# ericlingit/jieba-go

Measured on AMD Instinct MI355X. Metric: UTF-8 Chinese chars/sec segmented (whole node) + achieved HBM GB/s vs peak, higher is better.
Workload: dtype f64

## Files before the change

jieba-go_amd/csrc/jb_kernels.hip:

```cpp
#include <type_traits>

#include "jb_kdev.h"
#include "jb_kstages.h"

#include <algorithm>

namespace jb {

#define START_B (-0.26268660809250016)
#define START_S (-1.4652633398537678)
#define T_BE (-0.51082562376599)
#define T_BM (-0.916290731874155)
#define T_EB (-0.5897149736854513)
#define T_ES (-0.8085250474669937)
#define T_ME (-0.33344856811948514)
#define T_MM (-1.2603623820268226)
#define T_SB (-0.7211965654669841)
#define T_SS (-0.6658631448798212)

__global__ void k_docbits(const uint64_t* __restrict__ doc_off, uint32_t ndocs, uint64_t nbytes,
                          uint32_t* __restrict__ bits, uint32_t* __restrict__ counters,
                          uint64_t* __restrict__ tstat, uint32_t ntt) {
    const uint32_t d = blockIdx.x * blockDim.x + threadIdx.x;
    if (d < CNT_ALL) counters[d] = 0u;
    if (d < ntt) tstat[d] = 0ull;
    if (d >= ndocs) return;
    const uint64_t o = doc_off[d];
    if (o < nbytes) atomicOr(bits + (o >> 5), 1u << (o & 31u));
}

constexpr uint32_t kTileE = kTileBytes / 3 + 2;
constexpr uint32_t kLA = 8;
constexpr uint32_t kLABytes = 40;
constexpr uint32_t kTileEX = kTileE + kLA;
constexpr uint32_t kMwStage = kTileBytes + 64u;
constexpr uint32_t kMwOffE = kTileEX * 8u;
constexpr uint32_t kMwOffDb = kMwOffE + kTileEX * 4u;
constexpr uint32_t kMwOffWl = kMwOffDb + (kTileBytes / 32u + 3u) * 4u;
constexpr uint32_t kMwOffScan = (kMwOffWl + kTileE * 2u + 3u) & ~3u;
constexpr uint32_t kMwSortB = 64u;
constexpr uint32_t kMwOffHist = kMwOffScan + 8u * 4u;
constexpr uint32_t kMwLds = kMwOffHist + kMwSortB * 4u;
constexpr uint32_t kMwOffHot = (kMwOffE + 15u) & ~15u;
static_assert(kMwOffHot % 16u == 0u && kMwOffHot + 10u * JB_HOT_SLOTS <= kMwOffDb && JB_HOT_SLOTS == 512u,
              "k_mark_walk: the hot rows fit under the entry list, 256 threads stage them");
static_assert(kMwOffE >= kMwStage, "staged text must fit under the entry cells");
static_assert(kTileBytes + kLABytes + 4u <= kMwStage - 16u && kTileBytes + kLABytes + 4u <= kTileBytes + 64u,
              "lookahead bytes are staged and have document bits");
static_assert(kMwLds + 16u <= 163840u / 8u, "k_mark_walk: 8 workgroups per CU");

constexpr uint32_t kEntCont = 0x40000000u;
constexpr uint32_t kEntEdge = 0x80000000u;
__device__ __forceinline__ uint32_t ent_code(uint32_t e) { return e & 0x1FFFFu; }
__device__ __forceinline__ uint32_t ent_pos(uint32_t e) { return (e >> 18) & 0xFFFu; }
__device__ __forceinline__ uint32_t ent_w(uint32_t e) { return 3u + ((e >> 17) & 1u); }

#ifndef JB_MW_SGPR
#define JB_MW_SGPR 80
#endif
#ifndef JB_MW_WALKS
#define JB_MW_WALKS 1
#endif
#define JB_MW_ATTR __attribute__((amdgpu_num_sgpr(JB_MW_SGPR), amdgpu_waves_per_eu(8, 8)))
__global__ __launch_bounds__(256) JB_MW_ATTR void k_mark_walk(const uint8_t* __restrict__ text, uint64_t nbytes,
                                                   const uint32_t* __restrict__ docbits, DevImage im,
                                                   uint32_t* __restrict__ lanemask, uint2* __restrict__ tile_cnt,
                                                   uint64_t* __restrict__ erec, uint32_t* __restrict__ tile4,
                                                   uint64_t* __restrict__ alnum16, uint32_t* __restrict__ sbits,
                                                   uint32_t* __restrict__ ebits, uint32_t diag,
                                                   uint64_t* __restrict__ dbg, uint32_t split) {
    __shared__ __attribute__((aligned(16))) uint8_t s_raw[kMwLds];
    uint64_t* const s_c = reinterpret_cast<uint64_t*>(s_raw);
    uint8_t* const s_t = s_raw;
    uint32_t* const s_e = reinterpret_cast<uint32_t*>(s_raw + kMwOffE);
    uint32_t* const s_db = reinterpret_cast<uint32_t*>(s_raw + kMwOffDb);
    uint16_t* const s_wl = reinterpret_cast<uint16_t*>(s_raw + kMwOffWl);
    uint32_t* const lds = reinterpret_cast<uint32_t*>(s_raw + kMwOffScan);
    __shared__ uint32_t s_nla, s_nwl;
#if JB_STAMPS
    const bool stamps = (diag & 0x100u) != 0;
#else
    const bool stamps = false;
#endif
    uint64_t c0 = stamps ? __builtin_amdgcn_s_memtime() : 0, c1 = 0, c2 = 0, c3 = 0, c0b = 0, c1b = 0;
    uint32_t trips = 0;
    const uint32_t tile = blockIdx.x >> split, part = blockIdx.x & ((1u << split) - 1u);
    const uint64_t t0 = (uint64_t)tile * kTileBytes;
    static_assert(kMwStage / 16 > 256u && kMwStage / 16 <= 512u, "the staged text is two loads per thread at most");
    uint4 va = make_uint4(0, 0, 0, 0), vb = make_uint4(0, 0, 0, 0);
    {
        const int64_t g = (int64_t)t0 - 16 + 16 * (int64_t)threadIdx.x, g2 = g + 16 * 256;
        if (g >= 0 && (uint64_t)g + 16 <= nbytes + 64) va = *reinterpret_cast<const uint4*>(text + g);
        if (threadIdx.x < kMwStage / 16 - 256u && (uint64_t)g2 + 16 <= nbytes + 64)
            vb = *reinterpret_cast<const uint4*>(text + g2);
    }
    const uint4 hv4 = reinterpret_cast<const uint4*>(im.hot)[threadIdx.x];
    const uint32_t ht2 = reinterpret_cast<const uint32_t*>(im.hot + JB_HOT_SLOTS)[threadIdx.x];
    const uint64_t lastw = (nbytes + 31) >> 5;
    uint32_t dbw = 0;
    if (threadIdx.x < kTileBytes / 32 + 3) {
        const uint64_t wi = (t0 >> 5) + threadIdx.x;
        dbw = wi < lastw ? docbits[wi] : 0u;
    }
    if (threadIdx.x == 0) {
        s_nla = 0;
        s_nwl = 0;
    }
    uint32_t* const s_hist = reinterpret_cast<uint32_t*>(s_raw + kMwOffHist);
    if (threadIdx.x < kMwSortB) s_hist[threadIdx.x] = 0u;
    const uint64_t p0 = t0 + threadIdx.x * 16u;
    uint64_t M;
    {
        const int64_t base = (int64_t)p0 - 4;
        if (base >= 0) {
            const uint64_t wi = (uint64_t)base >> 5;
            const uint32_t off = (uint32_t)base & 31u;
            const uint64_t lo = wi < lastw ? docbits[wi] : 0u;
            const uint64_t hi = wi + 1 < lastw ? docbits[wi + 1] : 0u;
            M = ((hi << 32) | lo) >> off;
        } else {
            M = (uint64_t)docbits[0] << 4;
        }
        if (nbytes < p0 + 20) {
            const int64_t endk = (int64_t)nbytes - base;
            if (endk <= 0) M = ~0ull;
            else M |= ~0ull << endk;
        }
    }
    reinterpret_cast<uint4*>(s_t)[threadIdx.x] = va;
    if (threadIdx.x < kMwStage / 16 - 256u) reinterpret_cast<uint4*>(s_t)[threadIdx.x + 256u] = vb;
    if (threadIdx.x < kTileBytes / 32 + 3) s_db[threadIdx.x] = dbw;
    reinterpret_cast<uint4*>(s_raw + kMwOffHot)[threadIdx.x] = hv4;
    reinterpret_cast<uint32_t*>(s_raw + kMwOffHot + 8u * JB_HOT_SLOTS)[threadIdx.x] = ht2;
    {
        const uint64_t wz = (t0 >> 5) + (threadIdx.x & 127u);
        if (wz < lastw + 2u) __builtin_nontemporal_store(0u, (threadIdx.x < 128u ? sbits : ebits) + wz);
    }
    __syncthreads();
    if (stamps) c0b = __builtin_amdgcn_s_memtime();
    const uint8_t* win = s_t + 12 + threadIdx.x * 16u;
    uint32_t xw[5];
    {
        const uint4 v4 = *reinterpret_cast<const uint4*>(win + 4);
        xw[1] = v4.x;
        xw[2] = v4.y;
        xw[3] = v4.z;
        xw[4] = v4.w;
        uint32_t w0 = 0;
        if ((threadIdx.x & 63u) == 0u) w0 = reinterpret_cast<const uint32_t*>(win)[0];
        xw[0] = (uint32_t)__builtin_amdgcn_update_dpp((int)w0, (int)xw[4], 0x138, 0xF, 0xF, false);
    }
    {
        const bool al = ((uint32_t)jb_any_alnum4(xw[1]) | (uint32_t)jb_any_alnum4(xw[2]) |
                         (uint32_t)jb_any_alnum4(xw[3]) | (uint32_t)jb_any_alnum4(xw[4])) != 0u;
        const uint64_t am = __ballot(al);
        if ((threadIdx.x & 63u) == 0) alnum16[(t0 >> 10) + (threadIdx.x >> 6)] = am;
    }
    uint32_t lead = 0;
#pragma unroll
    for (int j = 0; j < 5; j++) {
        const uint32_t x = xw[j];
        const uint32_t f = (x & (x << 1) & 0x80808080u) >> 7;
        lead |= ((f * 0x204081u) >> 21 & 0xFu) << (4 * j);
    }
    uint32_t covered = 0, hanb = 0;
    uint64_t cl[7];
    uint32_t hsm = 0, kp = 0;
    uint32_t rowp[4] = {0u, 0u, 0u, 0u};
    {
        constexpr uint64_t k3000 = (1ull << 5) | (1ull << 7) | (0x1FFull << 0x21) | (0xFull << 0x38);
        uint32_t l = lead, slow = 0, xs[7], vm = 0;
        uint64_t kq = 0;
#pragma unroll
        for (int i = 0; i < 7; i++) {
            vm |= (l != 0u ? 1u : 0u) << i;
            const uint32_t k = l ? (uint32_t)__builtin_ctz(l) : 0u;
            kq |= (uint64_t)k << (5 * i);
            xs[i] = lds4(win, k);
            l &= l - 1u;
        }
#pragma unroll
        for (int i = 0; i < 7; i++) {
            const bool v = (vm >> i) & 1u;
            const uint32_t k = (uint32_t)(kq >> (5 * i)) & 31u, x = xs[i];
            const uint32_t b0 = x & 0xFFu;
            const uint32_t r = ((b0 & 0x0Fu) << 12) | (((x >> 8) & 0x3Fu) << 6) | ((x >> 16) & 0x3Fu);
            const bool plain = (b0 - 0xE1u < 12u) | (b0 - 0xEEu < 2u);
            const bool rare = (r - 0x2E80u < 0x180u) | (r - 0xF900u < 0x200u);
            const bool ok = ((x & 0x00C0C000u) == 0x00808000u) & (((uint32_t)(M >> (k + 1u)) & 3u) == 0u);
            const uint32_t o = r - 0x3000u;
            const bool h = (r - 0x4E00u <= 0x9FFCu - 0x4E00u) | (r - 0x3400u <= 0x4DBFu - 0x3400u) |
                           ((o < 64u) & (((k3000 >> (o & 63u)) & 1ull) != 0ull));
            const bool fast = plain & !(ok & rare);
            slow |= ((v & !fast) ? 1u : 0u) << k;
            covered |= ((v & fast & ok) ? 3u : 0u) << (k + 1u);
            hanb |= ((v & fast & ok & h) ? 7u : 0u) << k;
            const bool dr = v & fast & ok & h & (k >= 4u) & (r >= JB_DIRECT_LO);
            rowp[i >> 1] |= (dr ? r - 0x3300u : 0u) << (16 * (i & 1));
            hsm |= (dr ? 1u : 0u) << i;
            kp |= (dr ? k - 4u : 0u) << (4 * i);
        }
        slow |= l;
        lead = slow;
    }
    while (lead) {
        const uint32_t k = __builtin_ctz(lead);
        lead &= lead - 1u;
        const uint32_t lim = 1u + (uint32_t)__builtin_ctzll(((M >> (k + 1)) & 7ull) | 8ull);
        uint32_t r;
        const uint32_t w = dec_lead(lds4(win, k), lim, &r);
        covered |= ((1u << (w - 1u)) - 1u) << (k + 1u);
        if (w >= 3u && han_cp(r)) hanb |= ((1u << w) - 1u) << k;
    }
    if (p0 == 0) hanb &= ~0xFu;
    uint32_t valid = 0xFFFF0u;
    if (nbytes < p0 + 16) valid = nbytes > p0 ? ((1u << (uint32_t)(nbytes - p0)) - 1u) << 4 : 0u;
    const uint32_t bs = ~covered & valid & ((uint32_t)M | (hanb ^ (hanb << 1)));
    const uint32_t bmask = (bs >> 4) & 0xFFFFu, zmask = ((bs & hanb) >> 4) & 0xFFFFu;
    __builtin_nontemporal_store(bmask | (zmask << 16), lanemask + tile * 256u + threadIdx.x);
    uint32_t tot;
    block_scan_u32(__popc(bmask) | (__popc(zmask) << 16), lds, &tot);
    if (threadIdx.x == 0) tile_cnt[tile] = make_uint2(tot & 0xFFFFu, tot >> 16);
    if (stamps) c1 = __builtin_amdgcn_s_memtime();

    uint32_t hs = ((hanb & ~covered & valid) >> 4) & 0xFFFFu;
    {
        const uint64_t* s_hv = reinterpret_cast<const uint64_t*>(s_raw + kMwOffHot);
        const uint16_t* s_ht = reinterpret_cast<const uint16_t*>(s_raw + kMwOffHot + 8u * JB_HOT_SLOTS);
        uint32_t hit = 0, tg[7];
#pragma unroll
        for (int i = 0; i < 7; i++) {
            const uint32_t r = ((rowp[i >> 1] >> (16 * (i & 1))) & 0xFFFFu) + 0x3300u;
            tg[i] = s_ht[jb_hot_slot(r)];
            cl[i] = s_hv[jb_hot_slot(r)];
        }
#pragma unroll
        for (int i = 0; i < 7; i++) {
            const uint32_t r = ((rowp[i >> 1] >> (16 * (i & 1))) & 0xFFFFu) + 0x3300u;
            hit |= (((hsm >> i) & 1u) & (tg[i] == r ? 1u : 0u)) << i;
        }
#pragma unroll
        for (int i = 0; i < 7; i++) {
            const uint32_t row = (rowp[i >> 1] >> (16 * (i & 1))) & 0xFFFFu;
            if (!((hit >> i) & 1u)) cl[i] = 0ull;
            if ((~hit & hsm) >> i & 1u) cl[i] = im.l1row[row];
        }
    }
    uint32_t nent;
    uint32_t o = block_scan_u32(__popc(hs), lds, &nent);
    bool has4 = false;
    {
        uint32_t w4m = 0;
        if (__popc(hs) != __popc(hsm)) {
            const uint32_t ne = __popc(hs);
            uint32_t h2 = hs;
            hsm = 0;
            kp = 0;
#pragma unroll
            for (int i = 0; i < 6; i++) {
                cl[i] = 0ull;
                if ((uint32_t)i < ne) {
                    const uint32_t k = (uint32_t)__builtin_ctz(h2);
                    h2 &= h2 - 1u;
                    const uint32_t x = lds4(win, k + 4u);
                    const uint32_t r = (x & 0xF0u) == 0xE0u
                                           ? ((x & 0x0Fu) << 12) | (((x >> 8) & 0x3Fu) << 6) | ((x >> 16) & 0x3Fu)
                                           : ((x & 0x07u) << 18) | (((x >> 8) & 0x3Fu) << 12) |
                                                 (((x >> 16) & 0x3Fu) << 6) | ((x >> 24) & 0x3Fu);
                    cl[i] = im.l1row[jb_row(im.pagemap, r)];
                    hsm |= 1u << i;
                    kp |= k << (4 * i);
                    w4m |= (r >= 0x10000u ? 1u : 0u) << i;
                }
            }
            cl[6] = 0ull;
        }
        has4 = w4m != 0u;
        const uint32_t top = hsm ? 31u - (uint32_t)__builtin_clz(hsm) : 0u;
        const uint32_t lastend =
            hsm ? ((kp >> (4u * top)) & 15u) + 4u + 3u + ((w4m >> top) & 1u) : 0u;
        const uint32_t le255 = __builtin_amdgcn_readlane(lastend, 63);
        const bool la = threadIdx.x >= 192u && le255 >= 20u;
        uint32_t law = 0, lar = 0, lacd = 0;
        if (la) {
            const uint32_t j = threadIdx.x & 63u, q = kTileBytes + j;
            if (j < kLABytes) {
                const uint64_t db = ((((uint64_t)s_db[(q >> 5) + 1u]) << 32) | s_db[q >> 5]) >> (q & 31u);
                uint32_t lim = 1u + (uint32_t)__builtin_ctzll(((db >> 1) & 7ull) | 8ull);
                const uint64_t gq = t0 + q;
                if (gq + lim > nbytes) lim = gq < nbytes ? (uint32_t)(nbytes - gq) : 0u;
                lar = (db & 1ull) ? 0u : han_rune(lds4(s_t, q + 16u), lim, &law);
            }
            lacd = lar ? rune_code(im, lar) : 0u;
        }
#pragma unroll
        for (int i = 0; i < 7; i++) {
            if ((hsm >> i) & 1u)
                s_e[o + __popc(hsm & ((1u << i) - 1u))] = jb_l1row_code(cl[i]) | (((w4m >> i) & 1u) << 17) |
                                                          ((threadIdx.x * 16u + ((kp >> (4 * i)) & 15u)) << 18);
            cl[i] = ((hsm >> i) & 1u) ? jb_l1row_cell(cl[i]) : 0ull;
        }
        if (la) {
            const uint32_t j = threadIdx.x & 63u;
            const uint32_t w = law, r = lar, cdj = lacd;
            const uint64_t hm = __ballot(r != 0u), w4b = __ballot(w == 4u);
            uint64_t chain = 0;
            uint32_t jj = le255 - 20u, n = 0;
            bool go = true;
#pragma unroll
            for (int i = 0; i < (int)kLA; i++) {
                if (go && jj < kLABytes && ((hm >> jj) & 1ull)) {
                    chain |= 1ull << jj;
                    n++;
                    jj += ((w4b >> jj) & 1ull) ? 4u : 3u;
                } else {
                    go = false;
                }
            }
            if ((chain >> j) & 1ull) {
                const uint32_t ix = (uint32_t)__popcll(chain & ((1ull << j) - 1ull));
                s_e[nent + ix] = cdj | ((w == 4u ? 1u : 0u) << 17) | (ix + 1u < n ? kEntCont : (go ? kEntEdge : 0u));
            }
            if (j == 0u) s_nla = n;
        }
        __syncthreads();
        if (stamps) c1b = __builtin_amdgcn_s_memtime();
#pragma unroll
        for (int i = 0; i < 7; i++)
            if ((hsm >> i) & 1u) s_c[o + __popc(hsm & ((1u << i) - 1u))] = cl[i];
    }
    __syncthreads();
    const uint32_t nla = s_nla;
    uint32_t wm = 0;
    for (uint32_t i = threadIdx.x, k = 0; i < nent; i += 256u, k++) {
        const uint32_t e = s_e[i];
        const uint32_t nxt = ent_pos(e) + ent_w(e);
        uint32_t f = 0;
        if (nxt >= kTileBytes) f = nla ? kEntCont : 0u;
        else if (i + 1u < nent && ent_pos(s_e[i + 1u]) == nxt && !((s_db[nxt >> 5] >> (nxt & 31u)) & 1u)) f = kEntCont;
        s_e[i] = e | f;
        const uint64_t c1 = s_c[i];
        const uint32_t fc = jb_cell_fc(c1), wi = jb_cell_widx(c1);
        uint64_t r1 = 0;
        bool go = false;
        if (jb_cell_check(c1) != JB_CHECK_ROOT) {
            r1 = 1ull | ((uint64_t)(JB_WIDX_ABSENT + 1u) << kRecTop);
        } else if (wi > kRecIdxMax && fc != JB_FC_NEG) {
            r1 = 0ull;
        } else if (fc == JB_FC_ZERO) {
            r1 = 1ull | ((uint64_t)(wi + 1u) << kRecTop);
        } else {
            if (fc == JB_FC_POS) r1 = 1ull | ((uint64_t)(wi + 1u) << kRecTop);
            go = jb_cell_hc(c1) != 0u && f != 0u;
        }
        if (!im.plainw) {
            r1 = 0ull;
            go = false;
        }
        if (!go) {
            s_c[i] = r1;
        } else if (i < ((nent * part) >> split) || i >= ((nent * (part + 1u)) >> split)) {
        } else {
            const uint32_t ln = (jb_cell_base(c1) + ent_code(s_e[i + 1u])) >> 4;
            const uint32_t b = (ln * 0x9E3779B1u) >> 26;
            static_assert(kMwSortB == 64u && kTileEX <= 2048u, "bucket (6 bits) and rank (11 bits) in the check field");
            const uint32_t rk = atomicAdd(&s_hist[b], 1u);
            s_c[i] = (c1 & ~0x3FFFFFull) | (b << 11) | rk;
            wm |= 1u << k;
        }
    }
    const int any4 = __syncthreads_or(has4);
    if (threadIdx.x == 0) tile4[tile] = any4 ? 1u : 0u;
    if (threadIdx.x < 64u) {
        const uint32_t h = s_hist[threadIdx.x];
        const uint32_t x = wave_incl_scan(h);
        s_hist[threadIdx.x] = x - h;
        if (threadIdx.x == 63u) s_nwl = x;
    }
    __syncthreads();
    for (uint32_t k = 0; wm >> k; k++) {
        if ((wm >> k) & 1u) {
            const uint32_t i = threadIdx.x + 256u * k;
            const uint32_t ck = (uint32_t)s_c[i] & 0x3FFFFFu;
            s_wl[s_hist[ck >> 11] + (ck & 2047u)] = (uint16_t)i;
        }
    }
    __syncthreads();
    if (stamps) c2 = __builtin_amdgcn_s_memtime();
    const uint32_t* ent = s_e;
    const uint32_t wv = threadIdx.x >> 6;
    const uint32_t nwl = s_nwl;
    uint32_t head = (nwl * wv) >> 2;
    const uint32_t hi = (nwl * (wv + 1u)) >> 2;
    struct Walk {
        bool act, ovf;
        uint32_t j, js, id, base, len, nedge, m, en;
        uint64_t rw;
    };
    Walk wk[JB_MW_WALKS];
#pragma unroll
    for (int q = 0; q < JB_MW_WALKS; q++) {
        wk[q].act = wk[q].ovf = false;
        wk[q].j = wk[q].js = wk[q].id = wk[q].base = wk[q].len = wk[q].nedge = wk[q].m = wk[q].en = 0u;
        wk[q].rw = 0ull;
    }
    for (;;) {
#pragma unroll
        for (int q = 0; q < JB_MW_WALKS; q++) {
            Walk& w = wk[q];
            const uint64_t need = __ballot(!w.act);
            const uint32_t rank =
                __builtin_amdgcn_mbcnt_hi((uint32_t)(need >> 32), __builtin_amdgcn_mbcnt_lo((uint32_t)need, 0u));
            const uint32_t j0 = head + rank;
            const bool fresh = !w.act && j0 < hi;
            head = min(hi, head + (uint32_t)__popcll(need));
            if (fresh) {
                w.js = s_wl[j0];
                w.j = w.js;
                const uint64_t c = s_c[w.j];
                w.id = ent_code(ent[w.j]);
                w.base = jb_cell_base(c);
                const bool pos = jb_cell_fc(c) == JB_FC_POS;
                w.m = pos ? 1u : 0u;
                w.nedge = w.m;
                w.rw = pos ? (uint64_t)(jb_cell_widx(c) + 1u) << kRecTop : 0ull;
                w.len = 1u;
                w.ovf = false;
                w.act = true;
                w.en = ent[w.j + 1u];
            }
        }
        uint64_t child[JB_MW_WALKS];
        uint32_t tt[JB_MW_WALKS], en2[JB_MW_WALKS];
#pragma unroll
        for (int q = 0; q < JB_MW_WALKS; q++) {
            tt[q] = wk[q].base + ent_code(wk[q].en);
            child[q] = wk[q].act ? im.cells[tt[q]] : 0ull;
            en2[q] = ent[wk[q].j + 2u];
        }
#pragma unroll
        for (int q = 0; q < JB_MW_WALKS; q++) {
            Walk& w = wk[q];
            if (w.act) {
                const uint64_t ch = child[q];
                const bool hit = dat_hit(ch, w.id);
                ++w.len;
                const uint32_t wi = jb_cell_widx(ch);
                const bool pos = hit && jb_cell_fc(ch) == JB_FC_POS;
                const bool bad = pos && (w.len > kEdgeMaxL || w.nedge >= 4u || wi > kRecIdxMax);
                const bool add = pos && !bad;
                w.ovf |= bad;
                w.m |= add ? 1u << ((w.len - 1u) & 7u) : 0u;
                w.rw = add ? (w.rw >> kEdgeIdxBits) | ((uint64_t)(wi + 1u) << kRecTop) : w.rw;
                w.nedge += add ? 1u : 0u;
                const bool more = hit && jb_cell_hc(ch) && !w.ovf;
                const bool go = more && (w.en & kEntCont);
                const bool dfr = more && !(w.en & kEntCont) && (w.en & kEntEdge);
                ++w.j;
                w.en = en2[q];
                w.id = tt[q];
                w.base = jb_cell_base(ch);
                if (!go) {
                    s_c[w.js] = (w.ovf || dfr) ? 0ull : ((uint64_t)w.m | w.rw);
                    w.act = false;
                }
            }
        }
        trips++;
        bool any = false;
#pragma unroll
        for (int q = 0; q < JB_MW_WALKS; q++) any |= wk[q].act;
        if (!__any(any) && head >= hi) break;
    }
    if (stamps) c3 = __builtin_amdgcn_s_memtime();
    __syncthreads();
    {
        const uint32_t e0 = (nent * part) >> split, e1 = (nent * (part + 1u)) >> split;
        for (uint32_t i = e0 + threadIdx.x; i < e1; i += 256u)
            __builtin_nontemporal_store(s_c[i], erec + (t0 + ent_pos(s_e[i])) / 3u);
    }
    if (stamps && part == 0u && (threadIdx.x & 63u) == 0) {
        uint64_t* o = dbg + ((uint64_t)tile * 4u + (threadIdx.x >> 6)) * 8u;
        o[0] = c1 - c0;
        o[1] = c2 - c1;
        o[2] = c3 - c2;
        o[3] = __builtin_amdgcn_s_memtime() - c3;
        o[4] = trips;
        o[5] = 1;
        o[6] = c0b - c0;
        o[7] = c1b - c1;
    }
}

constexpr uint32_t kZhRing = 8;
#ifndef JB_ZH_SLACK
#define JB_ZH_SLACK 1024
#endif
#ifndef JB_ZH_CHUNK
#define JB_ZH_CHUNK 192
#endif
constexpr uint32_t kZhWin = kZhGroupBytes + JB_ZH_SLACK;
constexpr uint32_t kZhChunk = JB_ZH_CHUNK;
constexpr uint32_t kZhPer = kZhChunk / 64u;
static_assert(kZhChunk % 64u == 0u && kZhPer >= 1u && kZhPer <= 4u, "k_zh: 1-4 blocks per lane and chunk");
static_assert(kZhGroupBytes / 1024u + 1u <= 64u, "k_zh: a chunk's unresolved blocks fit the wave's 64 hist words");
constexpr uint32_t kZhWinWords = kZhWin / 32u + 1u;
static_assert(kZhGroupBytes % 32u == 0u && kZhGroupSmall % 32u == 0u && kZhGroupSmall <= kZhGroupBytes,
              "k_zh groups are whole token-bitmap words");
static_assert(2u * kZhWinWords <= 2u * kZhRing * 64u, "token bitmaps fit over the ring");
constexpr uint32_t kZhPool = 512u;
constexpr uint32_t kZhBlBytes = kZhWin / 3u + 4u;
static_assert(kZhWgWide * (((kZhBlBytes + 15u) & ~15u) + 8u * kZhRing * 64u + 4u * kZhChunk + 256u + 4u) + 2048u +
                      8u * kZhWtabWide <= 163840u,
              "k_zh wide form: LDS");
static_assert(kZhWin < 65536u, "window offsets are packed in 16 bits");
constexpr uint32_t kZhStageWords = kZhGroupBytes / 16u + 128u;
constexpr uint32_t kZhStagePer = (kZhStageWords + 63u) / 64u;
static_assert(kZhStagePer * 64u <= 2u * kZhRing * 64u,
              "k_zh: a group's lane-mask words and their lookahead must fit the wave's ring (JB_ZH_GROUP <= 14336)");

template <bool A3>
struct GrpZvT {
    static constexpr bool all3 = A3;
    const uint8_t* text;
    uint8_t* bls;
    uint32_t wb;
    __device__ __forceinline__ uint32_t b(uint32_t q) const { return text[q]; }
    __device__ __forceinline__ uint32_t x4(uint32_t q) const { return ld4(text, q); }
    __device__ __forceinline__ uint8_t& bl(uint32_t q) const { return bls[(q - wb) / 3u]; }
};
struct GlbZv {
    static constexpr bool all3 = false;
    const uint8_t* text;
    uint8_t* gbl;
    __device__ __forceinline__ uint32_t b(uint32_t q) const { return text[q]; }
    __device__ __forceinline__ uint32_t x4(uint32_t q) const { return ld4(text, q); }
    __device__ __forceinline__ uint8_t& bl(uint32_t q) const { return gbl[q / 3u]; }
};

template <class V>
__device__ __forceinline__ uint32_t z_dec(const V& v, uint32_t q, uint32_t* w) {
    const uint32_t x = v.x4(q);
    const uint32_t b0 = x & 0xFFu;
    if (V::all3 || b0 < 0xF0u) {
        *w = 3;
        return ((b0 & 0x0Fu) << 12) | (((x >> 8) & 0x3Fu) << 6) | ((x >> 16) & 0x3Fu);
    }
    *w = 4;
    return ((b0 & 0x07u) << 18) | (((x >> 8) & 0x3Fu) << 12) | (((x >> 16) & 0x3Fu) << 6) | ((x >> 24) & 0x3Fu);
}
template <class V>
__device__ __forceinline__ uint32_t z_w(const V& v, uint32_t q) {
    if (V::all3) return 3u;
    return v.b(q) < 0xF0u ? 3u : 4u;
}
template <class V>
__device__ __forceinline__ uint32_t z_prev(const V& v, uint32_t q, uint32_t lo) {
    if (V::all3) return q - 3u;
    if (q - lo < 4u) return lo;
    return (v.b(q - 3u) & 0xF0u) == 0xE0u ? q - 3u : q - 4u;
}

__device__ __forceinline__ void load_emit(const DevImage& im, uint32_t r, double e[4]) {
    const double2* p = reinterpret_cast<const double2*>(im.emit) + (size_t)jb_row(im.pagemap, r) * 2u;
    const double2 a = p[0], b = p[1];
    e[0] = a.x; e[1] = a.y; e[2] = b.x; e[3] = b.y;
}

__device__ __forceinline__ void route2(double a, double b, uint32_t* code, double* p, uint32_t& nt) {
    uint32_t c = 2u;
    double best = JB_MIN_FLOAT;
    if (a > best) { c = 0u; best = a; }
    if (b > best) { c = 1u; best = b; }
    nt += (a == b && a > JB_MIN_FLOAT) ? 1u : 0u;
    *code = c;
    *p = best;
}

template <class V, class E>
__device__ void viterbi_back(const V& v, uint32_t rs, uint32_t re, uint32_t m, uint32_t st, E& em) {
    uint32_t t = m - 1, reset = 0;
    uint32_t qt = z_prev(v, re, rs);
    for (;;) {
        if (t == 0) {
            v.bl(qt) = (uint8_t)st;
            break;
        }
        const uint32_t code = (v.bl(qt) >> (2u * st)) & 3u;
        v.bl(qt) = (uint8_t)st;
        if (code == 2u) {
            reset = t;
            break;
        }
        st = (st == JB_B || st == JB_S) ? 2u + code : code;
        --t;
        qt = z_prev(v, qt, rs);
    }
    uint32_t qa = rs, qb = qt, ts = rs;
    for (uint32_t k = 0; k < m - reset; k++) {
        const uint32_t lab = v.bl(qb);
        qa += z_w(v, qa);
        qb += z_w(v, qb);
        if (lab >= (uint32_t)JB_E) {
            em.token(ts, qa);
            ts = qa;
        }
    }
}

template <class V, class E>
__device__ void viterbi_run(const V& v, const DevImage& im, uint32_t rs, uint32_t re, uint32_t m, E& em) {
    if (m == 1) {
        em.token(rs, re);
        return;
    }
    uint32_t w;
    double e[4], en[4];
    uint32_t r = z_dec(v, rs, &w);
    load_emit(im, r, e);
    double vB = START_B + e[0], vM = JB_MIN_FLOAT + e[1], vE = JB_MIN_FLOAT + e[2], vS = START_S + e[3];
    uint32_t q = rs + w;
    if (q < re) load_emit(im, z_dec(v, q, &w), e);
    while (q < re) {
        const uint32_t qn = q + w;
        uint32_t wn = 0;
        if (qn < re) load_emit(im, z_dec(v, qn, &wn), en);
        uint32_t cB, cM, cE, cS;
        double pB, pM, pE, pS;
        route2(vE + T_EB, vS + T_SB, &cB, &pB, em.ties);
        route2(vB + T_BM, vM + T_MM, &cM, &pM, em.ties);
        route2(vB + T_BE, vM + T_ME, &cE, &pE, em.ties);
        route2(vE + T_ES, vS + T_SS, &cS, &pS, em.ties);
        vB = pB + e[0];
        vM = pM + e[1];
        vE = pE + e[2];
        vS = pS + e[3];
        v.bl(q) = (uint8_t)(cB | (cM << 2) | (cE << 4) | (cS << 6));
        q = qn;
        w = wn;
        e[0] = en[0]; e[1] = en[1]; e[2] = en[2]; e[3] = en[3];
    }
    viterbi_back(v, rs, re, m, vE > vS ? (uint32_t)JB_E : (uint32_t)JB_S, em);
}

struct TblSrc {
    const uint32_t* t;
    uint32_t nseg, wb;
    __device__ __forceinline__ bool next(uint32_t& j, uint32_t& bs, uint32_t& be) const {
        while (j < nseg) {
            const uint32_t x = t[j * 64u];
            j++;
            if (x != ~0u) {
                bs = wb + (x & 0xFFFFu);
                be = wb + (x >> 16);
                return true;
            }
        }
        return false;
    }
};
struct TblPeek {
    uint32_t bs, be;
    bool ok;
};
struct RegSrc {
    uint32_t x[kZhPer];
    uint32_t wb;
    __device__ __forceinline__ explicit RegSrc(const TblSrc& s) : wb(s.wb) {
#pragma unroll
        for (uint32_t i = 0; i < kZhPer; i++) x[i] = s.nseg > i ? s.t[64u * i] : ~0u;
    }
    __device__ __forceinline__ bool next(uint32_t& j, uint32_t& bs, uint32_t& be) {
        if (x[0] == ~0u) return false;
        j++;
        bs = wb + (x[0] & 0xFFFFu);
        be = wb + (x[0] >> 16);
#pragma unroll
        for (uint32_t i = 0; i + 1u < kZhPer; i++) x[i] = x[i + 1u];
        x[kZhPer - 1u] = ~0u;
        return true;
    }
};
__device__ __forceinline__ TblPeek tbl_peek(const RegSrc& src, uint32_t) {
    return TblPeek{src.wb + (src.x[0] & 0xFFFFu), src.wb + (src.x[0] >> 16), src.x[0] != ~0u};
}
struct OneSrc {
    uint32_t bs0, be0;
    __device__ __forceinline__ bool next(uint32_t& j, uint32_t& bs, uint32_t& be) const {
        if (j) return false;
        j = 1;
        bs = bs0;
        be = be0;
        return true;
    }
};

struct DpFold {
    double prevP = JB_MIN_FLOAT, bestP = JB_MIN_FLOAT;
    uint32_t bestL = 0, lastL = 0;
    bool redo = false;
    __device__ __forceinline__ void item(uint32_t L, double wt, uint32_t c, const double* ring, bool longm,
                                         const double* __restrict__ gbest, uint32_t key0) {
        double nb;
        if (L == c) nb = 0.0;
        else if (L <= kZhRing) nb = ring[((c - L) & (kZhRing - 1u)) * 64u];
        else if (longm) nb = gbest[key0 - (c - L)];
        else {
            redo = true;
            nb = 0.0;
        }
        const double pp = wt + nb;
        if (pp >= prevP) {
            bestL = L;
            bestP = pp;
        }
        prevP = pp;
        lastL = L;
    }
    __device__ __forceinline__ void finish() {
        if (bestL == 0) {
            bestL = lastL;
            bestP = prevP;
        }
    }
};

template <class V>
__device__ __forceinline__ void dp_walk_rune(const V& v, const DevImage& im, uint32_t q, uint32_t be, DpFold& f,
                                             uint32_t c, const double* ring, bool longm,
                                             const double* __restrict__ gbest, uint32_t key0) {
    uint32_t w0;
    const uint32_t r0 = z_dec(v, q, &w0);
    uint32_t id = rune_code(im, r0);
    uint64_t cc = im.cells[id];
    if (jb_cell_check(cc) != JB_CHECK_ROOT) {
        f.item(1u, im.wtab[JB_WIDX_ABSENT], c, ring, longm, gbest, key0);
    } else if (jb_cell_fc(cc) == JB_FC_ZERO) {
        f.item(1u, im.wtab[jb_cell_widx(cc)], c, ring, longm, gbest, key0);
    } else {
        if (jb_cell_fc(cc) == JB_FC_POS) f.item(1u, im.wtab[jb_cell_widx(cc)], c, ring, longm, gbest, key0);
        uint32_t qq = q + w0, len = 1;
        bool go = jb_cell_hc(cc) != 0u;
        while (go && qq < be) {
            uint32_t wr;
            const uint32_t r = z_dec(v, qq, &wr);
            const uint32_t tt = dat_slot(im, cc, r);
            const uint64_t ch = im.cells[tt];
            if (!dat_hit(ch, id)) break;
            ++len;
            qq += wr;
            if (jb_cell_fc(ch) == JB_FC_POS) f.item(len, im.wtab[jb_cell_widx(ch)], c, ring, longm, gbest, key0);
            go = jb_cell_hc(ch) != 0u;
            id = tt;
            cc = ch;
        }
    }
}

typedef const __attribute__((address_space(1))) char gchar;
typedef const __attribute__((address_space(3))) char lchar;
__shared__ __attribute__((aligned(32))) double s_wt[kZhWtabWide];
template <bool WL = false>
__device__ __forceinline__ void rec_weights(const DevImage& im, uint64_t rc, double w[4]) {
    gchar* const wb = (gchar*)im.wtab1;
#pragma unroll
    for (int k = 0; k < 4; k++) {
        const uint32_t off = (uint32_t)(rc >> (8 + kEdgeIdxBits * k - 3)) & (((1u << kEdgeIdxBits) - 1u) << 3);
        if constexpr (WL) w[k] = *(const __attribute__((address_space(3))) double*)((lchar*)s_wt + off);
        else w[k] = *(const __attribute__((address_space(1))) double*)(wb + off);
    }
}

__shared__ uint64_t s_ltab[256];
__device__ __forceinline__ uint64_t ltab_entry(uint32_t m) {
    uint32_t L[4] = {1u, 1u, 1u, 1u}, n = 0;
    for (uint32_t b = 0; b < 8u; b++)
        if ((m >> b) & 1u) {
            L[0] = L[1];
            L[1] = L[2];
            L[2] = L[3];
            L[3] = b + 1u;
            n++;
// ... 3370 lines not shown
```

Before: 57.75 billion.

## Slim k_mark_walk to 32-bit arithmetic, branchless stores, and a single-walk loop

Rewrites several parts of the mark-walk kernel to use 32-bit instead of 64-bit arithmetic: the document mask uses alignbit, the k-queue is split into two 32-bit words, and the walk record is kept as two 32-bit halves. Predicated LDS stores now go to a dump slot instead of branching, the cell flags are decoded inline, and the multi-walk struct is replaced by a single walk state with a shifting length bit and byte-offset addressing. The aim is to cut VGPR/SGPR pressure and instruction count in a latency-bound trie walk at a fixed 8 waves per EU. The risk is subtle bit-field mistakes and extra LDS for the dump cells.

```diff
diff --git a/jieba-go_amd/csrc/jb_kernels.hip b/jieba-go_amd/csrc/jb_kernels.hip
--- a/jieba-go_amd/csrc/jb_kernels.hip
+++ b/jieba-go_amd/csrc/jb_kernels.hip
@@ -40,7 +40,11 @@
 constexpr uint32_t kMwOffScan = (kMwOffWl + kTileE * 2u + 3u) & ~3u;
 constexpr uint32_t kMwSortB = 64u;
 constexpr uint32_t kMwOffHist = kMwOffScan + 8u * 4u;
-constexpr uint32_t kMwLds = kMwOffHist + kMwSortB * 4u;
+constexpr uint32_t kMwOffDump = kMwOffHist + kMwSortB * 4u;
+constexpr uint32_t kMwLds = kMwOffDump + 16u;
+constexpr uint32_t kMwDumpC = kMwOffDump / 8u;
+constexpr uint32_t kMwDumpE = (kMwOffDump + 8u - kMwOffE) / 4u;
+static_assert(kMwOffDump % 8u == 0u && (kMwOffDump + 8u - kMwOffE) % 4u == 0u, "the dump cells are aligned");
 constexpr uint32_t kMwOffHot = (kMwOffE + 15u) & ~15u;
 static_assert(kMwOffHot % 16u == 0u && kMwOffHot + 10u * JB_HOT_SLOTS <= kMwOffDb && JB_HOT_SLOTS == 512u,
               "k_mark_walk: the hot rows fit under the entry list, 256 threads stage them");
@@ -57,9 +61,6 @@
 
 #ifndef JB_MW_SGPR
 #define JB_MW_SGPR 80
-#endif
-#ifndef JB_MW_WALKS
-#define JB_MW_WALKS 1
 #endif
 #define JB_MW_ATTR __attribute__((amdgpu_num_sgpr(JB_MW_SGPR), amdgpu_waves_per_eu(8, 8)))
 __global__ __launch_bounds__(256) JB_MW_ATTR void k_mark_walk(const uint8_t* __restrict__ text, uint64_t nbytes,
@@ -109,22 +110,22 @@
     uint32_t* const s_hist = reinterpret_cast<uint32_t*>(s_raw + kMwOffHist);
     if (threadIdx.x < kMwSortB) s_hist[threadIdx.x] = 0u;
     const uint64_t p0 = t0 + threadIdx.x * 16u;
-    uint64_t M;
+    uint32_t M;
     {
         const int64_t base = (int64_t)p0 - 4;
         if (base >= 0) {
             const uint64_t wi = (uint64_t)base >> 5;
             const uint32_t off = (uint32_t)base & 31u;
-            const uint64_t lo = wi < lastw ? docbits[wi] : 0u;
-            const uint64_t hi = wi + 1 < lastw ? docbits[wi + 1] : 0u;
-            M = ((hi << 32) | lo) >> off;
+            const uint32_t lo = wi < lastw ? docbits[wi] : 0u;
+            const uint32_t hi = wi + 1 < lastw ? docbits[wi + 1] : 0u;
+            M = __builtin_amdgcn_alignbit(hi, lo, off);
         } else {
-            M = (uint64_t)docbits[0] << 4;
+            M = docbits[0] << 4;
         }
         if (nbytes < p0 + 20) {
             const int64_t endk = (int64_t)nbytes - base;
-            if (endk <= 0) M = ~0ull;
-            else M |= ~0ull << endk;
+            if (endk <= 0) M = ~0u;
+            else M |= ~0u << (uint32_t)endk;
         }
     }
     reinterpret_cast<uint4*>(s_t)[threadIdx.x] = va;
@@ -170,24 +171,24 @@
     {
         constexpr uint64_t k3000 = (1ull << 5) | (1ull << 7) | (0x1FFull << 0x21) | (0xFull << 0x38);
         uint32_t l = lead, slow = 0, xs[7], vm = 0;
-        uint64_t kq = 0;
+        uint32_t kq[2] = {0u, 0u};
 #pragma unroll
         for (int i = 0; i < 7; i++) {
             vm |= (l != 0u ? 1u : 0u) << i;
             const uint32_t k = l ? (uint32_t)__builtin_ctz(l) : 0u;
-            kq |= (uint64_t)k << (5 * i);
+            kq[i / 6] |= k << (5 * (i % 6));
             xs[i] = lds4(win, k);
             l &= l - 1u;
         }
 #pragma unroll
         for (int i = 0; i < 7; i++) {
             const bool v = (vm >> i) & 1u;
-            const uint32_t k = (uint32_t)(kq >> (5 * i)) & 31u, x = xs[i];
+            const uint32_t k = (kq[i / 6] >> (5 * (i % 6))) & 31u, x = xs[i];
             const uint32_t b0 = x & 0xFFu;
             const uint32_t r = ((b0 & 0x0Fu) << 12) | (((x >> 8) & 0x3Fu) << 6) | ((x >> 16) & 0x3Fu);
             const bool plain = (b0 - 0xE1u < 12u) | (b0 - 0xEEu < 2u);
             const bool rare = (r - 0x2E80u < 0x180u) | (r - 0xF900u < 0x200u);
-            const bool ok = ((x & 0x00C0C000u) == 0x00808000u) & (((uint32_t)(M >> (k + 1u)) & 3u) == 0u);
+            const bool ok = ((x & 0x00C0C000u) == 0x00808000u) & (((M >> (k + 1u)) & 3u) == 0u);
             const uint32_t o = r - 0x3000u;
             const bool h = (r - 0x4E00u <= 0x9FFCu - 0x4E00u) | (r - 0x3400u <= 0x4DBFu - 0x3400u) |
                            ((o < 64u) & (((k3000 >> (o & 63u)) & 1ull) != 0ull));
@@ -206,7 +207,7 @@
     while (lead) {
         const uint32_t k = __builtin_ctz(lead);
         lead &= lead - 1u;
-        const uint32_t lim = 1u + (uint32_t)__builtin_ctzll(((M >> (k + 1)) & 7ull) | 8ull);
+        const uint32_t lim = 1u + (uint32_t)__builtin_ctz(((M >> (k + 1u)) & 7u) | 8u);
         uint32_t r;
         const uint32_t w = dec_lead(lds4(win, k), lim, &r);
         covered |= ((1u << (w - 1u)) - 1u) << (k + 1u);
@@ -215,7 +216,7 @@
     if (p0 == 0) hanb &= ~0xFu;
     uint32_t valid = 0xFFFF0u;
     if (nbytes < p0 + 16) valid = nbytes > p0 ? ((1u << (uint32_t)(nbytes - p0)) - 1u) << 4 : 0u;
-    const uint32_t bs = ~covered & valid & ((uint32_t)M | (hanb ^ (hanb << 1)));
+    const uint32_t bs = ~covered & valid & (M | (hanb ^ (hanb << 1)));
     const uint32_t bmask = (bs >> 4) & 0xFFFFu, zmask = ((bs & hanb) >> 4) & 0xFFFFu;
     __builtin_nontemporal_store(bmask | (zmask << 16), lanemask + tile * 256u + threadIdx.x);
     uint32_t tot;
@@ -239,11 +240,12 @@
             const uint32_t r = ((rowp[i >> 1] >> (16 * (i & 1))) & 0xFFFFu) + 0x3300u;
             hit |= (((hsm >> i) & 1u) & (tg[i] == r ? 1u : 0u)) << i;
         }
+        const uint8_t* const l1row8 = reinterpret_cast<const uint8_t*>(im.l1row);
+        const uint32_t miss = hsm & ~hit;
 #pragma unroll
         for (int i = 0; i < 7; i++) {
             const uint32_t row = (rowp[i >> 1] >> (16 * (i & 1))) & 0xFFFFu;
-            if (!((hit >> i) & 1u)) cl[i] = 0ull;
-            if ((~hit & hsm) >> i & 1u) cl[i] = im.l1row[row];
+            if ((miss >> i) & 1u) cl[i] = *reinterpret_cast<const uint64_t*>(l1row8 + (row << 3));
         }
     }
     uint32_t nent;
@@ -295,10 +297,10 @@
         }
 #pragma unroll
         for (int i = 0; i < 7; i++) {
-            if ((hsm >> i) & 1u)
-                s_e[o + __popc(hsm & ((1u << i) - 1u))] = jb_l1row_code(cl[i]) | (((w4m >> i) & 1u) << 17) |
-                                                          ((threadIdx.x * 16u + ((kp >> (4 * i)) & 15u)) << 18);
-            cl[i] = ((hsm >> i) & 1u) ? jb_l1row_cell(cl[i]) : 0ull;
+            const bool on = (hsm >> i) & 1u;
+            s_e[on ? o + __popc(hsm & ((1u << i) - 1u)) : kMwDumpE] =
+                jb_l1row_code(cl[i]) | (((w4m >> i) & 1u) << 17) | ((threadIdx.x * 16u + ((kp >> (4 * i)) & 15u)) << 18);
+            cl[i] = jb_l1row_cell(cl[i]);
         }
         if (la) {
             const uint32_t j = threadIdx.x & 63u;
@@ -327,41 +329,34 @@
         if (stamps) c1b = __builtin_amdgcn_s_memtime();
 #pragma unroll
         for (int i = 0; i < 7; i++)
-            if ((hsm >> i) & 1u) s_c[o + __popc(hsm & ((1u << i) - 1u))] = cl[i];
+            s_c[((hsm >> i) & 1u) ? o + __popc(hsm & ((1u << i) - 1u)) : kMwDumpC] = cl[i];
     }
     __syncthreads();
     const uint32_t nla = s_nla;
     uint32_t wm = 0;
+    const uint32_t pe0 = (nent * part) >> split, pe1 = (nent * (part + 1u)) >> split;
+    const bool plainw = im.plainw != 0;
     for (uint32_t i = threadIdx.x, k = 0; i < nent; i += 256u, k++) {
-        const uint32_t e = s_e[i];
+        const uint32_t e = s_e[i], e1 = s_e[i + 1u];
+        const uint64_t c1 = s_c[i];
         const uint32_t nxt = ent_pos(e) + ent_w(e);
-        uint32_t f = 0;
-        if (nxt >= kTileBytes) f = nla ? kEntCont : 0u;
-        else if (i + 1u < nent && ent_pos(s_e[i + 1u]) == nxt && !((s_db[nxt >> 5] >> (nxt & 31u)) & 1u)) f = kEntCont;
-        s_e[i] = e | f;
-        const uint64_t c1 = s_c[i];
-        const uint32_t fc = jb_cell_fc(c1), wi = jb_cell_widx(c1);
-        uint64_t r1 = 0;
-        bool go = false;
-        if (jb_cell_check(c1) != JB_CHECK_ROOT) {
-            r1 = 1ull | ((uint64_t)(JB_WIDX_ABSENT + 1u) << kRecTop);
-        } else if (wi > kRecIdxMax && fc != JB_FC_NEG) {
-            r1 = 0ull;
-        } else if (fc == JB_FC_ZERO) {
-            r1 = 1ull | ((uint64_t)(wi + 1u) << kRecTop);
+        const uint32_t dbit = (s_db[nxt >> 5] >> (nxt & 31u)) & 1u;
+        const bool cont = nxt >= kTileBytes ? nla != 0u
+                                            : (i + 1u < nent) & (ent_pos(e1) == nxt) & (dbit == 0u);
+        s_e[i] = e | (cont ? kEntCont : 0u);
+        const uint32_t clo = (uint32_t)c1, chi = (uint32_t)(c1 >> 32);
+        const uint32_t fc = (chi >> 12) & 3u, wi1 = (chi >> 15) + 1u;
+        const bool root = (clo & 0x3FFFFFu) == JB_CHECK_ROOT;
+        const bool fits = !(wi1 > kRecIdxMax + 1u && fc != JB_FC_NEG);
+        const bool edge = plainw & (!root | (fits & ((fc == JB_FC_ZERO) | (fc == JB_FC_POS))));
+        const uint32_t r1lo = edge ? 1u : 0u;
+        const uint32_t r1hi = edge ? (root ? wi1 : JB_WIDX_ABSENT + 1u) << (kRecTop - 32u) : 0u;
+        const bool go = plainw & root & fits & (fc != JB_FC_ZERO) & ((chi & 0x4000u) != 0u) & cont;
+        if (!go) {
+            s_c[i] = ((uint64_t)r1hi << 32) | r1lo;
+        } else if (i < pe0 || i >= pe1) {
         } else {
-            if (fc == JB_FC_POS) r1 = 1ull | ((uint64_t)(wi + 1u) << kRecTop);
-            go = jb_cell_hc(c1) != 0u && f != 0u;
-        }
-        if (!im.plainw) {
-            r1 = 0ull;
-            go = false;
-        }
-        if (!go) {
-            s_c[i] = r1;
-        } else if (i < ((nent * part) >> split) || i >= ((nent * (part + 1u)) >> split)) {
-        } else {
-            const uint32_t ln = (jb_cell_base(c1) + ent_code(s_e[i + 1u])) >> 4;
+            const uint32_t ln = (jb_cell_base(c1) + ent_code(e1)) >> 4;
             const uint32_t b = (ln * 0x9E3779B1u) >> 26;
             static_assert(kMwSortB == 64u && kTileEX <= 2048u, "bucket (6 bits) and rank (11 bits) in the check field");
             const uint32_t rk = atomicAdd(&s_hist[b], 1u);
@@ -388,96 +383,75 @@
     __syncthreads();
     if (stamps) c2 = __builtin_amdgcn_s_memtime();
     const uint32_t* ent = s_e;
-    const uint32_t wv = threadIdx.x >> 6;
-    const uint32_t nwl = s_nwl;
+    const uint32_t wv = __builtin_amdgcn_readfirstlane(threadIdx.x >> 6);
+    const uint32_t nwl = __builtin_amdgcn_readfirstlane(s_nwl);
     uint32_t head = (nwl * wv) >> 2;
     const uint32_t hi = (nwl * (wv + 1u)) >> 2;
-    struct Walk {
-        bool act, ovf;
-        uint32_t j, js, id, base, len, nedge, m, en;
-        uint64_t rw;
-    };
-    Walk wk[JB_MW_WALKS];
-#pragma unroll
-    for (int q = 0; q < JB_MW_WALKS; q++) {
-        wk[q].act = wk[q].ovf = false;
-        wk[q].j = wk[q].js = wk[q].id = wk[q].base = wk[q].len = wk[q].nedge = wk[q].m = wk[q].en = 0u;
-        wk[q].rw = 0ull;
-    }
+    static_assert(kEdgeMaxL == 8u && kEdgeIdxBits == 14u && kRecTop == 50u, "the walk trip's 32-bit record halves");
+    const uint8_t* const cells8 = reinterpret_cast<const uint8_t*>(im.cells);
+    const uint8_t* const ent8 = reinterpret_cast<const uint8_t*>(s_e);
+    uint8_t* const sc8 = reinterpret_cast<uint8_t*>(s_c);
+    uint32_t ja = 0, js8 = 0, id1 = 0, base = 0, en = 0, m = 0, lbit = 0, rlo = 0, rhi = 0;
     for (;;) {
-#pragma unroll
-        for (int q = 0; q < JB_MW_WALKS; q++) {
-            Walk& w = wk[q];
-            const uint64_t need = __ballot(!w.act);
+        const uint64_t need = __ballot(lbit == 0u);
+        if (need != 0ull && head < hi) {
             const uint32_t rank =
                 __builtin_amdgcn_mbcnt_hi((uint32_t)(need >> 32), __builtin_amdgcn_mbcnt_lo((uint32_t)need, 0u));
             const uint32_t j0 = head + rank;
-            const bool fresh = !w.act && j0 < hi;
             head = min(hi, head + (uint32_t)__popcll(need));
-            if (fresh) {
-                w.js = s_wl[j0];
-                w.j = w.js;
-                const uint64_t c = s_c[w.j];
-                w.id = ent_code(ent[w.j]);
-                w.base = jb_cell_base(c);
+            if (lbit == 0u && j0 < hi) {
+                const uint32_t js = s_wl[j0];
+                ja = js * 4u;
+                js8 = js * 8u;
+                const uint64_t c = s_c[js];
+                id1 = ent_code(ent[js]) + 1u;
+                en = ent[js + 1u];
+                base = jb_cell_base(c);
                 const bool pos = jb_cell_fc(c) == JB_FC_POS;
-                w.m = pos ? 1u : 0u;
-                w.nedge = w.m;
-                w.rw = pos ? (uint64_t)(jb_cell_widx(c) + 1u) << kRecTop : 0ull;
-                w.len = 1u;
-                w.ovf = false;
-                w.act = true;
-                w.en = ent[w.j + 1u];
-            }
-        }
-        uint64_t child[JB_MW_WALKS];
-        uint32_t tt[JB_MW_WALKS], en2[JB_MW_WALKS];
-#pragma unroll
-        for (int q = 0; q < JB_MW_WALKS; q++) {
-            tt[q] = wk[q].base + ent_code(wk[q].en);
-            child[q] = wk[q].act ? im.cells[tt[q]] : 0ull;
-            en2[q] = ent[wk[q].j + 2u];
-        }
-#pragma unroll
-        for (int q = 0; q < JB_MW_WALKS; q++) {
-            Walk& w = wk[q];
-            if (w.act) {
-                const uint64_t ch = child[q];
-                const bool hit = dat_hit(ch, w.id);
-                ++w.len;
-                const uint32_t wi = jb_cell_widx(ch);
-                const bool pos = hit && jb_cell_fc(ch) == JB_FC_POS;
-                const bool bad = pos && (w.len > kEdgeMaxL || w.nedge >= 4u || wi > kRecIdxMax);
-                const bool add = pos && !bad;
-                w.ovf |= bad;
-                w.m |= add ? 1u << ((w.len - 1u) & 7u) : 0u;
-                w.rw = add ? (w.rw >> kEdgeIdxBits) | ((uint64_t)(wi + 1u) << kRecTop) : w.rw;
-                w.nedge += add ? 1u : 0u;
-                const bool more = hit && jb_cell_hc(ch) && !w.ovf;
-                const bool go = more && (w.en & kEntCont);
-                const bool dfr = more && !(w.en & kEntCont) && (w.en & kEntEdge);
-                ++w.j;
-                w.en = en2[q];
-                w.id = tt[q];
-                w.base = jb_cell_base(ch);
-                if (!go) {
-                    s_c[w.js] = (w.ovf || dfr) ? 0ull : ((uint64_t)w.m | w.rw);
-                    w.act = false;
-                }
+                m = pos ? 1u : 0u;
+                rlo = 0u;
+                rhi = pos ? (jb_cell_widx(c) + 1u) << (kRecTop - 32u) : 0u;
+                lbit = 2u;
+            }
+        }
+        if (lbit != 0u) {
+            const uint32_t tt = base + ent_code(en);
+            const uint64_t ch = *reinterpret_cast<const uint64_t*>(cells8 + (tt << 3));
+            const uint32_t en2 = *reinterpret_cast<const uint32_t*>(ent8 + ja + 8u);
+            const uint32_t clo = (uint32_t)ch, chi = (uint32_t)(ch >> 32);
+            const bool hit = (clo & 0x3FFFFFu) == id1;
+            const bool pos = hit && ((chi >> 12) & 3u) == JB_FC_POS;
+            const uint32_t wi1 = (chi >> 15) + 1u;
+            const bool bad = pos && (lbit > (1u << (kEdgeMaxL - 1u)) || (rlo & 0x3FFF00u) != 0u || wi1 > kRecIdxMax + 1u);
+            const bool add = pos && !bad;
+            m |= add ? lbit : 0u;
+            const uint32_t nlo = __builtin_amdgcn_alignbit(rhi, rlo, kEdgeIdxBits);
+            const uint32_t nhi = (rhi >> kEdgeIdxBits) | (wi1 << (kRecTop - 32u));
+            rlo = add ? nlo : rlo;
+            rhi = add ? nhi : rhi;
+            lbit = __builtin_elementwise_add_sat(lbit, lbit);
+            const bool more = hit && (chi & 0x4000u) != 0u && !bad;
+            const bool go = more && (en & kEntCont);
+            const bool dfr = more && !(en & kEntCont) && (en & kEntEdge);
+            id1 = tt + 1u;
+            base = __builtin_amdgcn_alignbit(chi, clo, 22) & 0x3FFFFFu;
+            ja += 4u;
+            en = en2;
+            if (!go) {
+                *reinterpret_cast<uint64_t*>(sc8 + js8) = (bad || dfr) ? 0ull : ((uint64_t)rhi << 32) | (rlo | m);
+                lbit = 0u;
             }
         }
         trips++;
-        bool any = false;
-#pragma unroll
-        for (int q = 0; q < JB_MW_WALKS; q++) any |= wk[q].act;
-        if (!__any(any) && head >= hi) break;
+        if (!__any(lbit != 0u) && head >= hi) break;
     }
     if (stamps) c3 = __builtin_amdgcn_s_memtime();
     __syncthreads();
     {
-        const uint32_t e0 = (nent * part) >> split, e1 = (nent * (part + 1u)) >> split;
-        for (uint32_t i = e0 + threadIdx.x; i < e1; i += 256u)
-            __builtin_nontemporal_store(s_c[i], erec + (t0 + ent_pos(s_e[i])) / 3u);
+        uint64_t* const erec0 = erec + t0 / 3u;
+        const uint32_t r0 = (uint32_t)(t0 % 3u);
+        for (uint32_t i = pe0 + threadIdx.x; i < pe1; i += 256u)
+            __builtin_nontemporal_store(s_c[i], erec0 + (r0 + ent_pos(s_e[i])) / 3u);
     }
     if (stamps && part == 0u && (threadIdx.x & 63u) == 0) {
         uint64_t* o = dbg + ((uint64_t)tile * 4u + (threadIdx.x >> 6)) * 8u;
```

Result: faster. 59.90 billion (median of 6 runs) (+3.7%).
